# ideafisher/ssUnet-GAN

Hardware: AMD Instinct MI355X
Metric: train images/sec (512^2 tiles) (higher is better)
Workload: dtype f32; 1 GPU; UNet_R_SS_v2 generator + SRGAN-style discriminator, one G+D step (train_seg_gan.py:182-233), 16 x 3x512x512 tiles per GPU, fp32, Adam lr 2e-5; global_batch=16, tile=512, parallelism=dp1, dead_d_param_grads_of_g_step=computed

## Files before the change

ssunet-gan_amd/csrc/bn.hip:

```cpp
#include "common.h"

namespace {

constexpr int RED_BLOCK = 256;
constexpr int MAX_PARTS = 1024;

struct RedGeom { int TQ, PR, groups, parts; long long rows_per_part; };

__host__ RedGeom red_geom(long long P, int C, int Q = 1) {
  RedGeom g;
  const int CQ = (C + 4 * Q - 1) / (4 * Q);
  g.TQ = CQ >= 64 ? 64 : 1;
  if (CQ < 64) { while (g.TQ < CQ) g.TQ <<= 1; }
  g.PR = RED_BLOCK / g.TQ;
  g.groups = (CQ + g.TQ - 1) / g.TQ;
  long long parts = (P + (long long)g.PR * 8 - 1) / ((long long)g.PR * 8);
  if (parts > MAX_PARTS) parts = MAX_PARTS;
  if (parts < 1) parts = 1;
  g.rows_per_part = (P + parts - 1) / parts;
  g.parts = (int)((P + g.rows_per_part - 1) / g.rows_per_part);
  return g;
}

template <int MODE, typename T, bool BITS = false>
// ... 115 lines not shown
    double* dst = part + (size_t)blockIdx.x * 2 * Cpad;
#pragma unroll
    for (int e = 0; e < V; ++e) { dst[V * cg + e] = a1[e]; dst[Cpad + V * cg + e] = a2[e]; }
  }
}

__global__ __launch_bounds__(RED_BLOCK) void modulate_bwd_sums_kernel(
    const float* __restrict__ x, int ldx, const float* __restrict__ gb, int ldgb, const float* __restrict__ dy, int lddy,
    long long P, int C, float* __restrict__ dx, int lddx, float* __restrict__ dgb, int lddgb,
    int TQ, int PR, long long rows_per_part, double* __restrict__ part ) {
  __shared__ double red[2][RED_BLOCK][4];
  const int tid = threadIdx.x;
  const int tq = tid % TQ, pr = tid / TQ;
  const int cq = blockIdx.y * TQ + tq;
  const int CQ = C / 4;
  const bool cok = cq < CQ;
  const long long p0 = (long long)blockIdx.x * rows_per_part;
  long long p1 = p0 + rows_per_part; if (p1 > P) p1 = P;
  double s1[4] = {0, 0, 0, 0}, s2[4] = {0, 0, 0, 0};
  if (cok) {
    for (long long p = p0 + pr; p < p1; p += PR) {
      const f32x4 xv = *(const f32x4*)(x + p * ldx + 4 * cq);
      const f32x4 g = *(const f32x4*)(gb + p * ldgb + 4 * cq);
      const f32x4 d = *(const f32x4*)(dy + p * lddy + 4 * cq);
      const f32x4 dg = d * xv;
      st4(dx + p * lddx + 4 * cq, d * (1.f + g));
      st4(dgb + p * lddgb + 4 * cq, dg);
      st4(dgb + p * lddgb + C + 4 * cq, d);
#pragma unroll
      for (int e = 0; e < 4; ++e) { s1[e] += (double)dg[e]; s2[e] += (double)d[e]; }
    }
  }
#pragma unroll
  for (int e = 0; e < 4; ++e) { red[0][tid][e] = s1[e]; red[1][tid][e] = s2[e]; }
  __syncthreads();
  if (pr == 0 && cok) {
    double a1[4] = {0, 0, 0, 0}, a2[4] = {0, 0, 0, 0};
    for (int r = 0; r < PR; ++r)
#pragma unroll
      for (int e = 0; e < 4; ++e) { a1[e] += red[0][r * TQ + tq][e]; a2[e] += red[1][r * TQ + tq][e]; }
    double* dst = part + (size_t)blockIdx.x * 2 * C;
#pragma unroll
    for (int e = 0; e < 4; ++e) { dst[4 * cq + e] = a1[e]; dst[C + 4 * cq + e] = a2[e]; }
  }
}

__global__ __launch_bounds__(RED_BLOCK) void modulate_dgamma_sums_kernel(
    const float* __restrict__ x, int ldx, const float* __restrict__ dy, int lddy, long long P, int C,
    float* __restrict__ dg_out, int lddg, int TQ, int PR, long long rows_per_part, double* __restrict__ part ) {
  __shared__ double red[2][RED_BLOCK][4];
  const int tid = threadIdx.x;
  const int tq = tid % TQ, pr = tid / TQ;
  const int cq = blockIdx.y * TQ + tq;
  const int CQ = C / 4;
  const bool cok = cq < CQ;
  const long long p0 = (long long)blockIdx.x * rows_per_part;
  long long p1 = p0 + rows_per_part; if (p1 > P) p1 = P;
  double s1[4] = {0, 0, 0, 0}, s2[4] = {0, 0, 0, 0};
  if (cok) {
    for (long long p = p0 + pr; p < p1; p += PR) {
      const f32x4 xv = *(const f32x4*)(x + p * ldx + 4 * cq);
      const f32x4 d = *(const f32x4*)(dy + p * lddy + 4 * cq);
      const f32x4 dg = d * xv;
      st4(dg_out + p * lddg + 4 * cq, dg);
#pragma unroll
      for (int e = 0; e < 4; ++e) { s1[e] += (double)dg[e]; s2[e] += (double)d[e]; }
    }
  }
#pragma unroll
  for (int e = 0; e < 4; ++e) { red[0][tid][e] = s1[e]; red[1][tid][e] = s2[e]; }
  __syncthreads();
  if (pr == 0 && cok) {
    double a1[4] = {0, 0, 0, 0}, a2[4] = {0, 0, 0, 0};
    for (int r = 0; r < PR; ++r)
#pragma unroll
      for (int e = 0; e < 4; ++e) { a1[e] += red[0][r * TQ + tq][e]; a2[e] += red[1][r * TQ + tq][e]; }
    double* dst = part + (size_t)blockIdx.x * 2 * C;
#pragma unroll
    for (int e = 0; e < 4; ++e) { dst[4 * cq + e] = a1[e]; dst[C + 4 * cq + e] = a2[e]; }
  }
}

constexpr int FIN_LANES = 32;

struct BnFin {
  const float* weight; const float* bias; float eps, momentum; int var_mode;
  float* running_mean; float* running_var; float* mean; float* invstd; float* scale; float* shift;
};

__device__ __forceinline__ void bn_finalize_channel(int c, double s1, double s2, double count, const BnFin& f) {
  const double m = s1 / count;
  double var = fma(-m, m, s2 / count);
  if (var < 0) var = 0;
  double is;
  if (f.var_mode == 0) is = 1.0 / sqrt(var + (double)f.eps);
  else is = 1.0 / sqrt(var < (double)f.eps ? (double)f.eps : var);
  const float mf = (float)m, isf = (float)is;
  f.mean[c] = mf; f.invstd[c] = isf;
  const float w = f.weight ? f.weight[c] : 1.f, b = f.bias ? f.bias[c] : 0.f;
  const float sc = w * isf;
  f.scale[c] = sc; f.shift[c] = fmaf(-mf, sc, b);
  if (f.running_mean) f.running_mean[c] = fmaf(f.momentum, mf, (1.f - f.momentum) * f.running_mean[c]);
  if (f.running_var) {
    const double unb = count > 1 ? var * count / (count - 1) : var;
    f.running_var[c] = fmaf(f.momentum, (float)unb, (1.f - f.momentum) * f.running_var[c]);
  }
}

__global__ __launch_bounds__(32 * FIN_LANES) void col_reduce_final_kernel(const double* __restrict__ part, int parts, int C, int C4,
                                                                          double* __restrict__ sums, float* __restrict__ fsum,
                                                                          double count_out, BnFin fin, double fin_count) {
  __shared__ double red[2][FIN_LANES][32];
  const int cl = threadIdx.x & 31, lane = threadIdx.x >> 5;
  const int c = blockIdx.x * 32 + cl;
  double a1 = 0, a2 = 0;
  if (c < C) {
#pragma unroll 4
    for (int b = lane; b < parts; b += FIN_LANES) { a1 += part[(size_t)b * 2 * C4 + c]; a2 += part[(size_t)b * 2 * C4 + C4 + c]; }
  }
  red[0][lane][cl] = a1; red[1][lane][cl] = a2;
  __syncthreads();
  if (lane == 0 && c < C) {
    double t1 = 0, t2 = 0;
#pragma unroll
    for (int k = 0; k < FIN_LANES; ++k) { t1 += red[0][k][cl]; t2 += red[1][k][cl]; }
    if (sums) { sums[c] = t1; sums[C + c] = t2; }
    if (fsum) fsum[c] = (float)t1;
    if (fin.mean) bn_finalize_channel(c, t1, t2, fin_count, fin);
  }
  if (sums && count_out > 0 && blockIdx.x == 0 && threadIdx.x == 0) sums[2 * C] = count_out;
}

__global__ void bn_finalize_kernel(const double* __restrict__ sums, double count_arg, int C, BnFin fin) {
  const int c = blockIdx.x * blockDim.x + threadIdx.x;
  if (c >= C) return;
  const double count = count_arg > 0 ? count_arg : sums[2 * C];
  bn_finalize_channel(c, sums[c], sums[C + c], count, fin);
}

template <typename T>
__global__ __launch_bounds__(256) void bn_apply_kernel(const T* __restrict__ x, long long P, int C, int ld,
                                                       const float* __restrict__ scale, const float* __restrict__ shift,
                                                       const T* __restrict__ res, int ldr, int act, float slope,
                                                       T* __restrict__ y, int ldy) {
  constexpr int Q = SsgQ<T>::value;
  const int CG = C / (4 * Q);
  const long long total = P * CG;
  SSG_CHUNK_LOOP(i, total) {
    const long long p = i / CG; const int c0 = 4 * Q * (int)(i - p * CG);
    f32x4 xv[Q], rv[Q], o[Q];
    ldq(x + p * ld + c0, xv);
    if (res) ldq(res + p * ldr + c0, rv);
#pragma unroll
    for (int q = 0; q < Q; ++q) {
      const f32x4 sc = *(const f32x4*)(scale + c0 + 4 * q), sh = *(const f32x4*)(shift + c0 + 4 * q);
      f32x4 v = xv[q] * sc + sh;
      if (res) v += rv[q];
#pragma unroll
      for (int e = 0; e < 4; ++e) v[e] = ssg_act(v[e], act, slope);
      o[q] = v;
    }
    stq(y + p * ldy + c0, o);
  }
}

__global__ __launch_bounds__(256) void bn_apply_mask_kernel(const float* __restrict__ x, long long P, int C, int ld,
                                                            const float* __restrict__ scale, const float* __restrict__ shift,
                                                            const float* __restrict__ res, int ldr, int act, float slope,
                                                            float* __restrict__ y, int ldy, uint8_t* __restrict__ mask, int ldm) {
  const int CG = C / 4;
  const long long total = P * CG;
  SSG_CHUNK_LOOP(i, total) {
    const long long p = i / CG; const int cq = (int)(i - p * CG); const int c0 = 4 * cq;
    const f32x4 xv = *(const f32x4*)(x + p * ld + c0);
    f32x4 rv = f32x4{0.f, 0.f, 0.f, 0.f};
    if (res) rv = *(const f32x4*)(res + p * ldr + c0);
    const f32x4 sc = *(const f32x4*)(scale + c0), sh = *(const f32x4*)(shift + c0);
    f32x4 v = xv * sc + sh;
    if (res) v += rv;
    unsigned nib = 0;
#pragma unroll
    for (int e = 0; e < 4; ++e) {
      v[e] = ssg_act(v[e], act, slope);
      nib |= (v[e] > 0.f ? 1u : 0u) << e;
    }
    st4(y + p * ldy + c0, v);
    const unsigned other = (unsigned)__builtin_amdgcn_mov_dpp((int)nib, 0xB1, 0xf, 0xf, false);
    if (!(cq & 1)) mask[p * ldm + (cq >> 1)] = (uint8_t)(nib | (other << 4));
  }
}

__device__ __forceinline__ float bn_dx_elem(float g, float xv, double k_mean, double k_is, double k_ws, double k_m1, double k_m2) {
  const double xh = ((double)xv - k_mean) * k_is;
  return (float)(k_ws * fma(-xh, k_m2, (double)g - k_m1));
}
__device__ __forceinline__ float bn_dx_elem(float g, float xv, float k_mean, float k_is, float k_ws, float k_m1, float k_m2) {
  const float xh = (xv - k_mean) * k_is;
  return k_ws * fmaf(-xh, k_m2, g - k_m1);
}

template <typename T, bool BITS = false>
// ... 572 lines not shown
```

ssunet-gan_amd/csrc/conv_wgrad.hip:

```cpp
#include "common.h"
#include "conv_thin.h"
#include "conv_wgrad_args.h"

namespace {

constexpr int BKP = 16;

template <int BM, int BN, int WAVES_M, int WAVES_N>
__global__ __launch_bounds__(256) void wgrad_kernel(const WgArgs a) {
  constexpr int WTM = BM / WAVES_M, WTN = BN / WAVES_N;
  constexpr int MI = WTM / 32, NI = WTN / 32;
  constexpr int LDA = BM + 4, LDB = BN + 4;
  constexpr int AQ = BM / 4, BQ = BN / 4;
  constexpr int A_LD = BKP * AQ / 256, B_LD = (BKP * BQ + 255) / 256;
  constexpr int A_PSTEP = 256 / AQ, B_PSTEP = 256 / BQ;
  static_assert(A_LD >= 1, "tile");

  __shared__ __attribute__((aligned(16))) float lds[2 * BKP * (LDA + LDB)];
  float* As = lds;
  float* Bs = lds + 2 * BKP * LDA;

  const int tid = threadIdx.x, lane = tid & 63, wave = tid >> 6;
  const int wm = wave / WAVES_N, wn = wave % WAVES_N;
  const int half = lane >> 5, l31 = lane & 31;
// ... 53 lines not shown
  };

  f32x16 acc[MI][NI];
#pragma unroll
  for (int i = 0; i < MI; ++i)
#pragma unroll
    for (int j = 0; j < NI; ++j)
#pragma unroll
      for (int r = 0; r < 16; ++r) acc[i][j][r] = 0.f;

  if (nsteps > 0) {
    load_step(0);
    store_step(0);
  }
  __syncthreads();
  for (int s = 0; s < nsteps; ++s) {
    const int buf = s & 1;
    const bool more = (s + 1) < nsteps;
    if (more) load_step(s + 1);
    const float* Ab = As + buf * BKP * LDA + half * LDA + wm * WTM + l31;
    const float* Bb = Bs + buf * BKP * LDB + half * LDB + wn * WTN + l31;
#pragma unroll
    for (int kk = 0; kk < BKP / 2; ++kk) {
      float fa[MI], fb[NI];
#pragma unroll
      for (int i = 0; i < MI; ++i) fa[i] = Ab[2 * kk * LDA + i * 32];
#pragma unroll
      for (int j = 0; j < NI; ++j) fb[j] = Bb[2 * kk * LDB + j * 32];
#pragma unroll
      for (int i = 0; i < MI; ++i)
#pragma unroll
        for (int j = 0; j < NI; ++j)
          acc[i][j] = __builtin_amdgcn_mfma_f32_32x32x2f32(fa[i], fb[j], acc[i][j], 0, 0, 0);
    }
    if (more) store_step(buf ^ 1);
    __syncthreads();
  }

  float* slab = a.ws + (size_t)blockIdx.z * a.M * a.Cout;
#pragma unroll
  for (int i = 0; i < MI; ++i)
#pragma unroll
    for (int j = 0; j < NI; ++j) {
      const int co = n0 + wn * WTN + j * 32 + l31;
#pragma unroll
      for (int r = 0; r < 16; ++r) {
        const int row = m0 + wm * WTM + i * 32 + (r & 3) + 8 * (r >> 2) + 4 * half;
        if (row < a.M && co < a.Cout) slab[(size_t)row * a.Cout + co] = acc[i][j][r];
      }
    }
}

struct RedArgs {
  const float* ws; float* dw; int splits, M, Cout, Cin, Cin_real, KH, KW, ntaps;
  int ky[SSG_MAX_TAPS], kx[SSG_MAX_TAPS];
};

template <int ZL>
__global__ __launch_bounds__(32 * ZL) void wgrad_reduce_kernel(const RedArgs a) {
  __shared__ float red[ZL][32];
  const int el = threadIdx.x & 31, zl = threadIdx.x >> 5;
  const long long idx = (long long)blockIdx.x * 32 + el;
  const long long tot = (long long)a.M * a.Cout;
  float s = 0.f;
  if (idx < tot) {
    int z = zl;
    for (; z + 3 * ZL < a.splits; z += 4 * ZL) {
      const float v0 = a.ws[(size_t)z * tot + idx], v1 = a.ws[(size_t)(z + ZL) * tot + idx];
      const float v2 = a.ws[(size_t)(z + 2 * ZL) * tot + idx], v3 = a.ws[(size_t)(z + 3 * ZL) * tot + idx];
      s += v0; s += v1; s += v2; s += v3;
    }
    for (; z < a.splits; z += ZL) s += a.ws[(size_t)z * tot + idx];
  }
  red[zl][el] = s;
  __syncthreads();
  if (zl != 0 || idx >= tot) return;
  float v = 0.f;
#pragma unroll
  for (int k = 0; k < ZL; ++k) v += red[k][el];
  const int row = (int)(idx / a.Cout), co = (int)(idx - (long long)row * a.Cout);
  const int t = row / a.Cin, c = row - t * a.Cin;
  if (c >= a.Cin_real) return;
  a.dw[(((size_t)co * a.Cin_real + c) * a.KH + a.ky[t]) * a.KW + a.kx[t]] = v;
}

enum { WG_MFMA, WG_HALO, WG_K32, WG_4 };
struct Plan { int variant, mt, nt, splits, steps_per_split, kind; };

bool wgrad_uses_dma(int variant) { return variant <= 1; }

bool wgrad_uses_halo(const ssg_wgrad_desc* d, int variant) { return wgrad_uses_dma(variant) && ssg_wgrad_halo_ok(d, variant); }

Plan make_plan(const ssg_wgrad_desc* d) {
  Plan p;
  p.kind = WG_MFMA;
  if (const int w4 = ssg_wgrad4_kind(d)) {
    p.kind = WG_4; p.variant = w4;
    p.mt = p.nt = p.steps_per_split = 0;
    p.splits = ssg_wgrad4_slices(d, w4, nullptr, nullptr, nullptr);
    return p;
  }
  const int Cin = d->C1 + d->C2;
  const int M = d->ntaps * Cin;
  int bn;
  if (d->Cout > 64) { p.variant = 0; bn = 128; }
  else if (d->Cout > 32) { p.variant = 1; bn = 64; }
  else { p.variant = 2; bn = 32; }
  p.mt = (M + 127) / 128;
  p.nt = (d->Cout + bn - 1) / bn;
  long long steps = ((long long)d->N * d->GH * d->GW + BKP - 1) / BKP;
  if (wgrad_uses_halo(d, p.variant)) {
    p.kind = WG_HALO;
    p.mt = Cin / ssg_wgrad_halo_cb(p.variant);
    steps = (long long)d->N * d->GH * ((d->GW + BKP - 1) / BKP);
  }
  if ((d->flags & 1) && ssg_wgrad_k32_ok(d)) {
    p.kind = WG_K32;
    p.mt = Cin / 64; p.nt = d->Cout / 64;
    steps = ssg_wgrad_k32_steps(d);
    const long long tiles = (long long)p.mt * p.nt;
    long long max_rows = 128;
    {
      const long long steps16 = (long long)d->N * d->GH * ((d->GW + BKP - 1) / BKP);
      const long long mtf = Cin / ssg_wgrad_halo_cb(p.variant), ntf = (d->Cout + (p.variant == 0 ? 127 : 63)) / (p.variant == 0 ? 128 : 64);
      long long wantf = 1024 / (mtf * ntf > 0 ? mtf * ntf : 1);
      if (wantf < 1) wantf = 1;
      if (wantf > steps16 / 16) wantf = steps16 / 16 > 0 ? steps16 / 16 : 1;
      if (wantf > 512) wantf = 512;
      const long long chain_px = (steps16 + wantf - 1) / wantf * BKP;
      if (chain_px / 32 < max_rows) max_rows = chain_px / 32;
      if (max_rows < 8) max_rows = 8;
    }
    const WgSlabs s = ssg_wgrad_slabs(steps, tiles, 8, max_rows);
    p.steps_per_split = s.steps_per_split; p.splits = s.splits;
    return p;
  }
  long long want = 1024 / ((long long)p.mt * p.nt);
  if (want < 1) want = 1;
  long long maxs = steps / 16;
  if (maxs < 1) maxs = 1;
  if (want > maxs) want = maxs;
  if (want > 512) want = 512;
  p.steps_per_split = (int)((steps + want - 1) / want);
  p.splits = (int)((steps + p.steps_per_split - 1) / p.steps_per_split);
  return p;
}

int validate(const ssg_wgrad_desc* d) {
  SSG_REQUIRE(d && d->in1 && d->dout && d->dw_oihw, SSG_EINVAL, "wgrad: null pointer");
  SSG_REQUIRE(d->C1 > 0 && d->C1 % 4 == 0 && d->C2 >= 0 && d->C2 % 4 == 0, SSG_EINVAL, "wgrad: channels must be multiples of 4");
  SSG_REQUIRE(d->C2 == 0 || d->in2, SSG_EINVAL, "wgrad: C2 > 0 needs in2");
  SSG_REQUIRE(d->ld1 % 4 == 0 && d->ld1 >= d->C1 && d->ldd % 4 == 0 && d->ldd >= d->Cout, SSG_EALIGN, "wgrad: strides");
  SSG_REQUIRE(d->C2 == 0 || (d->ld2 % 4 == 0 && d->ld2 >= d->C2), SSG_EALIGN, "wgrad: ld2");
  SSG_REQUIRE(ssg_aligned16(d->in1) && ssg_aligned16(d->in2) && ssg_aligned16(d->dout) && ssg_aligned16(d->ws), SSG_EALIGN, "wgrad: alignment");
  SSG_REQUIRE(d->ntaps >= 1 && d->ntaps <= SSG_MAX_TAPS, SSG_EINVAL, "wgrad: ntaps");
  SSG_REQUIRE(d->Cin_real > 0 && d->Cin_real <= d->C1 + d->C2, SSG_EINVAL, "wgrad: Cin_real");
  for (int t = 0; t < d->ntaps; ++t) {
    SSG_REQUIRE(d->dy[t] >= -2 && d->dy[t] <= 5 && d->dx[t] >= -2 && d->dx[t] <= 5, SSG_EINVAL, "wgrad: tap offset");
    SSG_REQUIRE(d->ky[t] >= 0 && d->ky[t] < d->KH && d->kx[t] >= 0 && d->kx[t] < d->KW, SSG_EINVAL, "wgrad: kernel position");
  }
  return SSG_OK;
}

int64_t workspace_bytes(const ssg_wgrad_desc* d, const Plan& p) {
  return (int64_t)p.splits * d->ntaps * (d->C1 + d->C2) * d->Cout * (int64_t)sizeof(float);
}
// ... 15 lines not shown
    const int span = ntaps * 16;
    const int chunk = k / span, rem = k - chunk * span;
    t = rem >> 4; c = chunk * 16 + (rem & 15);
  } else {
    t = k / Cred_pad; c = k - t * Cred_pad;
  }
  const int Cred = transpose ? O : I;
  float v = 0.f;
  if (t < ntaps && c < Cred) {
    const int kb = (int)((kpos_bits >> (6 * t)) & 63ull);
    const int ky = kb & 7, kx = kb >> 3;
    const int o = transpose ? c : r, i = transpose ? r : c;
    v = w[(((size_t)o * I + i) * KH + ky) * KW + kx];
    if (sigma) v *= 1.f / *sigma;
  }
  out[idx] = v;
}

}

WgArgs ssg_wgrad_args(const ssg_wgrad_desc* d, int steps_per_split) {
  WgArgs a;
  a.in1 = d->in1; a.in2 = d->C2 ? d->in2 : d->in1; a.dout = d->dout; a.ws = d->ws;
  a.C1 = d->C1; a.C2 = d->C2; a.ld1 = d->ld1; a.ld2 = d->C2 ? d->ld2 : d->ld1;
  a.N = d->N; a.H = d->H; a.W = d->W; a.Cout = d->Cout; a.ldd = d->ldd; a.GH = d->GH; a.GW = d->GW;
  a.in_sy = d->in_sy; a.in_sx = d->in_sx; a.ntaps = d->ntaps;
  a.tap_bits = ssg_pack_taps(d->dy, d->dx, d->ntaps);
  a.in_scale = d->in_scale; a.in_shift = d->in_shift; a.in_act = d->in_act; a.in_slope = d->in_slope;
  a.M = d->ntaps * (d->C1 + d->C2);
  a.Ptot = (long long)d->N * d->GH * d->GW;
  a.steps_per_split = steps_per_split;
  a.xcd_swizzle = 0;
  return a;
}

extern "C" int64_t ssg_conv2d_wgrad_workspace_bytes(const ssg_wgrad_desc* d) {
  return d ? workspace_bytes(d, make_plan(d)) : 0;
}

extern "C" int ssg_conv2d_wgrad_in_affine_ok(const ssg_wgrad_desc* d) {
  if (!d || !d->in1 || !d->dout) return 0;
  return in_affine_ok(d, make_plan(d)) ? 1 : 0;
}

extern "C" int ssg_conv2d_wgrad_f32(const ssg_wgrad_desc* d, void* stream) {
  int rc = validate(d);
  if (rc != SSG_OK) return rc;
  const Plan p = make_plan(d);
  SSG_REQUIRE(d->ws_bytes >= workspace_bytes(d, p), SSG_EINVAL, "wgrad: workspace too small");
  SSG_REQUIRE(!d->in_scale || (d->in_shift && in_affine_ok(d, p)), SSG_EINVAL,
              "wgrad: in_scale on a descriptor whose kernel has no fused input transform (ssg_conv2d_wgrad_in_affine_ok == 0)");
  hipStream_t st = (hipStream_t)stream;
  WgArgs a = ssg_wgrad_args(d, p.steps_per_split);
  if (p.kind == WG_4) {
    rc = ssg_wgrad4_launch(d, p.variant, st);
    if (rc != SSG_OK) return rc;
  } else {
    dim3 grid((unsigned)p.mt, (unsigned)p.nt, (unsigned)p.splits);
    if (p.kind == WG_K32) {
      rc = ssg_wgrad_k32_launch(a, grid, st);
      if (rc != SSG_OK) return rc;
    } else if (p.kind == WG_HALO) {
      rc = ssg_wgrad_halo_launch(a, p.variant, grid, st, (d->flags & 1) != 0);
      if (rc != SSG_OK) return rc;
    } else if (wgrad_uses_dma(p.variant)) {
      rc = ssg_wgrad_dma_launch(a, p.variant, grid, st, (d->flags & 1) != 0);
      if (rc != SSG_OK) return rc;
    } else {
      hipLaunchKernelGGL((wgrad_kernel<128, 32, 4, 1>), grid, dim3(256), 0, st, a);
    }
    SSG_LAUNCH_CHECK();
  }
  return ssg_wgrad_reduce_launch(d, p.splits, st);
}

int ssg_wgrad_reduce_launch(const ssg_wgrad_desc* d, int splits, hipStream_t st) {
  RedArgs r;
  r.ws = d->ws; r.dw = d->dw_oihw; r.splits = splits; r.M = d->ntaps * (d->C1 + d->C2); r.Cout = d->Cout; r.Cin = d->C1 + d->C2;
  r.Cin_real = d->Cin_real; r.KH = d->KH; r.KW = d->KW; r.ntaps = d->ntaps;
  for (int t = 0; t < SSG_MAX_TAPS; ++t) { r.ky[t] = t < d->ntaps ? d->ky[t] : 0; r.kx[t] = t < d->ntaps ? d->kx[t] : 0; }
  const long long tot = (long long)r.M * d->Cout;
  if (splits >= 256 && tot <= 32 * 1024)
    hipLaunchKernelGGL(wgrad_reduce_kernel<32>, dim3((unsigned)ssg_cdiv(tot, 32)), dim3(1024), 0, st, r);
  else
    hipLaunchKernelGGL(wgrad_reduce_kernel<8>, dim3((unsigned)ssg_cdiv(tot, 32)), dim3(256), 0, st, r);
  SSG_LAUNCH_CHECK();
  return SSG_OK;
}

extern "C" int ssg_pack_weights_scaled_f32(const float* w_oihw, int O, int I, int KH, int KW, int transpose, int ntaps,
                                           const int* ky, const int* kx, int kmode, int Cred_pad, int Kp, const float* sigma, float* out,
                                           void* stream);
extern "C" int ssg_pack_weights_f32(const float* w_oihw, int O, int I, int KH, int KW, int transpose, int ntaps,
                                    const int* ky, const int* kx, int kmode, int Cred_pad, int Kp, float* out,
                                    void* stream) {
  return ssg_pack_weights_scaled_f32(w_oihw, O, I, KH, KW, transpose, ntaps, ky, kx, kmode, Cred_pad, Kp, nullptr, out, stream);
}
extern "C" int ssg_pack_weights_scaled_f32(const float* w_oihw, int O, int I, int KH, int KW, int transpose, int ntaps,
                                           const int* ky, const int* kx, int kmode, int Cred_pad, int Kp, const float* sigma, float* out,
                                           void* stream) {
  SSG_REQUIRE(w_oihw && out && ky && kx, SSG_EINVAL, "pack: null pointer");
  SSG_REQUIRE(ntaps >= 1 && ntaps <= SSG_MAX_TAPS && KH <= 8 && KW <= 8, SSG_EINVAL, "pack: taps");
  SSG_REQUIRE(Kp % 16 == 0 && Cred_pad % 4 == 0, SSG_EINVAL, "pack: Kp/Cred_pad");
  const int Cred = transpose ? O : I;
  SSG_REQUIRE(Cred_pad >= Cred, SSG_EINVAL, "pack: Cred_pad < reduced channels");
  if (kmode == 0) SSG_REQUIRE(Cred_pad % 16 == 0 && Kp == ntaps * Cred_pad, SSG_EINVAL, "pack: kmode 0 shape");
  else SSG_REQUIRE(Kp >= ntaps * Cred_pad, SSG_EINVAL, "pack: kmode 1 Kp");
  unsigned long long bits = 0;
  for (int t = 0; t < ntaps; ++t) {
    SSG_REQUIRE(ky[t] >= 0 && ky[t] < KH && kx[t] >= 0 && kx[t] < KW, SSG_EINVAL, "pack: kernel position");
    bits |= (unsigned long long)(ky[t] | (kx[t] << 3)) << (6 * t);
  }
  const int R = transpose ? I : O;
  const long long tot = (long long)R * Kp;
  hipLaunchKernelGGL(pack_weights_kernel, dim3((unsigned)ssg_cdiv(tot, 256)), dim3(256), 0, (hipStream_t)stream,
                     w_oihw, O, I, KH, KW, transpose, ntaps, bits, kmode, Cred_pad, Kp, R, out, sigma);
  SSG_LAUNCH_CHECK();
  return SSG_OK;
}

extern "C" int ssg_conv2d_wgrad_kernel_id(const ssg_wgrad_desc* d) {
  if (!d) return SSG_EINVAL;
  const Plan p = make_plan(d);
  if (p.kind == WG_4) return 10 + p.variant;
  if (p.kind == WG_K32) return 60;
  if (p.kind == WG_HALO) return ((d->flags & 1) ? 40 : 30) + p.variant;
  return p.variant + (wgrad_uses_dma(p.variant) ? ((d->flags & 1) ? 50 : 20) : 0);
}

extern "C" int ssg_wgrad_dma_body(const ssg_wgrad_desc* d) {
  if (!d || validate(d) != SSG_OK) return 0;
  const Plan p = make_plan(d);
  if (p.kind != WG_MFMA || !wgrad_uses_dma(p.variant) || !(d->flags & 1)) return 0;
  return ssg_wgrad_dma_split_body(ssg_wgrad_args(d, p.steps_per_split), p.variant, (long long)p.mt * p.nt * p.splits);
}
```

ssunet-gan_amd/csrc/spatial.hip:

```cpp
#include "common.h"

namespace {

int elem_grid(long long total) { return ssg_elem_grid(total, 2); }

#define GRID_STRIDE(i, total) SSG_CHUNK_LOOP(i, total)

__global__ __launch_bounds__(256) void maxpool_fwd_kernel(const float* __restrict__ x, int N, int H, int W, int C, int ldx,
                                                          float* __restrict__ y, int ldy, uint8_t* __restrict__ idx) {
  const int OH = H / 2, OW = W / 2, CQ = C / 4;
  const long long total = (long long)N * OH * OW * CQ;
  GRID_STRIDE(i, total) {
    const int cq = (int)(i % CQ); long long r = i / CQ;
    const int ox = (int)(r % OW); r /= OW;
    const int oy = (int)(r % OH); const int n = (int)(r / OH);
    const float* b = x + ((size_t)(n * H + 2 * oy) * W + 2 * ox) * ldx + 4 * cq;
    f32x4 best = *(const f32x4*)b;
    int bi[4] = {0, 0, 0, 0};
#pragma unroll
    for (int k = 1; k < 4; ++k) {
      const f32x4 v = *(const f32x4*)(b + ((size_t)(k >> 1) * W + (k & 1)) * ldx);
#pragma unroll
      for (int e = 0; e < 4; ++e)
        if (v[e] > best[e] || v[e] != v[e]) { best[e] = v[e]; bi[e] = k; }
// ... 185 lines not shown
  int xlo, xhi;
  cand_range(ix, sx, OW, xlo, xhi);
  int oxf = -1, cnt = 0; float wx[5] = {0.f, 0.f, 0.f, 0.f, 0.f};
  for (int ox = xlo; ox <= xhi; ++ox) {
    int x0, x1; float lx0, lx1;
    lerp_coord(ox, sx, W, x0, x1, lx0, lx1);
    if (x0 != ix && x1 != ix) continue;
    if (oxf < 0) oxf = ox;
    const float wgt = (x0 == ix ? lx0 : 0.f) + (x1 == ix ? lx1 : 0.f);
    const int k = ox - oxf;
    if (k < 5) cnt = k + 1;
#pragma unroll
    for (int q = 0; q < 5; ++q) if (q == k) wx[q] = wgt;
  }
  const int b0 = band * BIL_BWD_BAND, b1 = min(b0 + BIL_BWD_BAND, H);
  int oylo, oyhi, t;
  cand_range(b0, sy, OH, oylo, t);
  cand_range(b1 - 1, sy, OH, t, oyhi);
  const float* src = dy + ((size_t)n * OH * OW + (oxf < 0 ? 0 : oxf)) * lddy + c4;
  float* dst = dx + ((size_t)n * H * W + ix) * lddx + c4;
  auto flush = [&](int r, const f32x4& v) { if (r >= b0 && r < b1) *(f32x4*)(dst + (size_t)r * W * lddx) = v; };
  int y0, y1; float ly0, ly1;
  lerp_coord(oylo, sy, H, y0, y1, ly0, ly1);
  int cur = y0;
  f32x4 acc0 = {0, 0, 0, 0}, acc1 = {0, 0, 0, 0};
  for (int oy = oylo; oy <= oyhi; ++oy) {
    lerp_coord(oy, sy, H, y0, y1, ly0, ly1);
    const float* row = src + (size_t)oy * OW * lddy;
    f32x4 h = {0, 0, 0, 0};
#pragma unroll
    for (int q = 0; q < 5; ++q)
      if (q < cnt) h += wx[q] * *(const f32x4*)(row + (size_t)q * lddy);
    if (y0 > cur) { flush(cur, acc0); acc0 = acc1; acc1 = f32x4{0, 0, 0, 0}; cur = y0; }
    acc0 += ly0 * h;
    if (y1 != y0) acc1 += ly1 * h; else acc0 += ly1 * h;
  }
  flush(cur, acc0);
  flush(cur + 1, acc1);
}

__global__ __launch_bounds__(256) void nearest_fwd_kernel(const float* __restrict__ x, int N, int H, int W, int C, int ldx,
                                                          float* __restrict__ y, int ldy) {
  const int OH = 2 * H, OW = 2 * W, CQ = C / 4;
  const long long total = (long long)N * OH * OW * CQ;
  GRID_STRIDE(i, total) {
    const int cq = (int)(i % CQ); long long r = i / CQ;
    const int ox = (int)(r % OW); r /= OW;
    const int oy = (int)(r % OH); const int n = (int)(r / OH);
    *(f32x4*)(y + ((size_t)(n * OH + oy) * OW + ox) * ldy + 4 * cq) =
        *(const f32x4*)(x + ((size_t)(n * H + (oy >> 1)) * W + (ox >> 1)) * ldx + 4 * cq);
  }
}
__global__ __launch_bounds__(256) void nearest_bwd_kernel(const float* __restrict__ dy, int lddy, int N, int H, int W, int C,
                                                          float* __restrict__ dx, int lddx) {
  const int OW = 2 * W, CQ = C / 4;
  const long long total = (long long)N * H * W * CQ;
  GRID_STRIDE(i, total) {
    const int cq = (int)(i % CQ); long long r = i / CQ;
    const int ix = (int)(r % W); r /= W;
    const int iy = (int)(r % H); const int n = (int)(r / H);
    const float* b = dy + ((size_t)(n * 2 * H + 2 * iy) * OW + 2 * ix) * lddy + 4 * cq;
    const f32x4 s = (*(const f32x4*)b + *(const f32x4*)(b + lddy)) + (*(const f32x4*)(b + (size_t)OW * lddy) + *(const f32x4*)(b + (size_t)(OW + 1) * lddy));
    *(f32x4*)(dx + ((size_t)(n * H + iy) * W + ix) * lddx + 4 * cq) = s;
  }
}

__device__ __forceinline__ int bin_lo(int o, int in, int out) { return (o * in) / out; }
__device__ __forceinline__ int bin_hi(int o, int in, int out) { return ((o + 1) * in + out - 1) / out; }

__global__ __launch_bounds__(256) void avgpool_flat_fwd_kernel(const float* __restrict__ x, int N, int H, int W, int C, int ldx,
                                                               int O, float* __restrict__ y) {
  const long long total = (long long)N * O * O * C;
  GRID_STRIDE(i, total) {
    const int c = (int)(i % C); long long r = i / C;
    const int ox = (int)(r % O); r /= O;
    const int oy = (int)(r % O); const int n = (int)(r / O);
    const int y0 = bin_lo(oy, H, O), y1 = bin_hi(oy, H, O), x0 = bin_lo(ox, W, O), x1 = bin_hi(ox, W, O);
    float s = 0.f;
    for (int yy = y0; yy < y1; ++yy)
      for (int xx = x0; xx < x1; ++xx) s += x[((size_t)(n * H + yy) * W + xx) * ldx + c];
    y[(size_t)n * C * O * O + (size_t)c * O * O + oy * O + ox] = s / (float)((y1 - y0) * (x1 - x0));
  }
}
__global__ __launch_bounds__(256) void avgpool_flat_bwd_kernel(const float* __restrict__ dy, int N, int H, int W, int C, int O,
                                                               float* __restrict__ dx, int lddx) {
  const long long total = (long long)N * H * W * C;
  GRID_STRIDE(i, total) {
    const int c = (int)(i % C); long long r = i / C;
    const int xx = (int)(r % W); r /= W;
    const int yy = (int)(r % H); const int n = (int)(r / H);
    float s = 0.f;
    for (int oy = 0; oy < O; ++oy) {
      const int y0 = bin_lo(oy, H, O), y1 = bin_hi(oy, H, O);
      if (yy < y0 || yy >= y1) continue;
      for (int ox = 0; ox < O; ++ox) {
        const int x0 = bin_lo(ox, W, O), x1 = bin_hi(ox, W, O);
        if (xx < x0 || xx >= x1) continue;
        s += dy[(size_t)n * C * O * O + (size_t)c * O * O + oy * O + ox] / (float)((y1 - y0) * (x1 - x0));
      }
    }
    dx[((size_t)(n * H + yy) * W + xx) * lddx + c] = s;
  }
}

__global__ __launch_bounds__(256) void nchw_to_nhwc_kernel(const float* __restrict__ src, int C, long long S, float* __restrict__ dst, int ld) {
  const long long p = (long long)blockIdx.x * 64 + (threadIdx.x & 63);
  const int n = blockIdx.y;
  if (p >= S) return;
  for (int c = threadIdx.x >> 6; c < ld; c += 4) {
    const float v = c < C ? src[((size_t)n * C + c) * S + p] : 0.f;
    dst[((size_t)n * S + p) * ld + c] = v;
  }
}
__global__ __launch_bounds__(256) void nhwc_to_nchw_kernel(const float* __restrict__ src, int ld, int C, long long S, float* __restrict__ dst) {
  const long long p = (long long)blockIdx.x * 64 + (threadIdx.x & 63);
  const int n = blockIdx.y;
  if (p >= S) return;
  for (int c = threadIdx.x >> 6; c < C; c += 4) dst[((size_t)n * C + c) * S + p] = src[((size_t)n * S + p) * ld + c];
}

static bool bilinear_stream_ok(int N, int H, int W, int C) {
  return C % 16 == 0 && H >= 3 && W >= 3 && (long long)N * (2 * H / BIL_FWD_BAND + 1) * (2 * W / 16 + 1) * (C / 16) < (1ll << 31);
}
#define REQ_Q(C, ...) SSG_REQUIRE((C) > 0 && (C) % 4 == 0, SSG_EINVAL, __VA_ARGS__)

}

extern "C" int ssg_maxpool2x2_fwd_f32(const float* x, int N, int H, int W, int C, int ldx, float* y, int ldy, uint8_t* idx, void* stream) {
  SSG_REQUIRE(x && y && idx && N > 0 && H >= 2 && W >= 2, SSG_EINVAL, "maxpool: bad args");
  REQ_Q(C, "maxpool: C %% 4");
  SSG_REQUIRE(ldx % 4 == 0 && ldy % 4 == 0, SSG_EALIGN, "maxpool: strides");
  const long long total = (long long)N * (H / 2) * (W / 2) * (C / 4);
  hipLaunchKernelGGL(maxpool_fwd_kernel, dim3(elem_grid(total)), dim3(256), 0, (hipStream_t)stream, x, N, H, W, C, ldx, y, ldy, idx);
  SSG_LAUNCH_CHECK();
  return SSG_OK;
}
extern "C" int ssg_maxpool2x2_bwd_f32(const float* dy, int lddy, const uint8_t* idx, int N, int H, int W, int C, float* dx, int lddx, void* stream) {
  SSG_REQUIRE(dy && dx && idx && N > 0 && H % 2 == 0 && W % 2 == 0, SSG_EINVAL, "maxpool_bwd: needs even H, W");
  REQ_Q(C, "maxpool_bwd: C %% 4");
  const long long total = (long long)N * (H / 2) * (W / 2) * (C / 4);
  hipLaunchKernelGGL(scatter2x2_kernel, dim3(elem_grid(total)), dim3(256), 0, (hipStream_t)stream, dy, lddy, idx, N, H / 2, W / 2, C, dx, lddx, (const float*)nullptr, 0);
  SSG_LAUNCH_CHECK();
  return SSG_OK;
}
extern "C" int ssg_maxpool2x2_bwd_add_f32(const float* dy, int lddy, const uint8_t* idx, const float* res, int ldr, int N, int H, int W, int C,
                                         float* dx, int lddx, void* stream) {
  SSG_REQUIRE(dy && dx && idx && res && N > 0 && H % 2 == 0 && W % 2 == 0 && ldr % 4 == 0, SSG_EINVAL, "maxpool_bwd_add: bad args");
  REQ_Q(C, "maxpool_bwd_add: C %% 4");
  const long long total = (long long)N * (H / 2) * (W / 2) * (C / 4);
  hipLaunchKernelGGL(scatter2x2_kernel, dim3(elem_grid(total)), dim3(256), 0, (hipStream_t)stream, dy, lddy, idx, N, H / 2, W / 2, C, dx, lddx, res, ldr);
  SSG_LAUNCH_CHECK();
  return SSG_OK;
}
extern "C" int ssg_maxunpool2x2_fwd_f32(const float* x, int ldx, const uint8_t* idx, int N, int OH, int OW, int C, float* y, int ldy, void* stream) {
  SSG_REQUIRE(x && y && idx && N > 0 && OH % 2 == 0 && OW % 2 == 0, SSG_EINVAL, "maxunpool: bad args");
  REQ_Q(C, "maxunpool: C %% 4");
  const long long total = (long long)N * (OH / 2) * (OW / 2) * (C / 4);
  hipLaunchKernelGGL(scatter2x2_kernel, dim3(elem_grid(total)), dim3(256), 0, (hipStream_t)stream, x, ldx, idx, N, OH / 2, OW / 2, C, y, ldy, (const float*)nullptr, 0);
  SSG_LAUNCH_CHECK();
  return SSG_OK;
}
extern "C" int ssg_maxunpool2x2_bwd_f32(const float* dy, int lddy, const uint8_t* idx, int N, int OH, int OW, int C, float* dx, int lddx, void* stream) {
  SSG_REQUIRE(dy && dx && idx && N > 0 && OH % 2 == 0 && OW % 2 == 0, SSG_EINVAL, "maxunpool_bwd: bad args");
  REQ_Q(C, "maxunpool_bwd: C %% 4");
  const long long total = (long long)N * (OH / 2) * (OW / 2) * (C / 4);
  hipLaunchKernelGGL(gather2x2_kernel, dim3(elem_grid(total)), dim3(256), 0, (hipStream_t)stream, dy, lddy, idx, N, OH / 2, OW / 2, C, dx, lddx);
  SSG_LAUNCH_CHECK();
  return SSG_OK;
}
extern "C" int ssg_upsample2x_bilinear_fwd_f32(const float* x, int N, int H, int W, int C, int ldx, float* y, int ldy, void* stream) {
  SSG_REQUIRE(x && y && N > 0 && H > 0 && W > 0, SSG_EINVAL, "bilinear: bad args");
  REQ_Q(C, "bilinear: C %% 4");
  const float sy = (2 * H > 1) ? (float)(H - 1) / (float)(2 * H - 1) : 0.f, sx = (2 * W > 1) ? (float)(W - 1) / (float)(2 * W - 1) : 0.f;
  SSG_REQUIRE((long long)N * 2 * H < (1ll << 31) && (long long)2 * W * (C / 4) < (1ll << 31), SSG_EINVAL, "bilinear: too large");
  if (bilinear_stream_ok(N, H, W, C)) {
    const int cqt = C % 64 == 0 ? 16 : C % 32 == 0 ? 8 : 4;
    const int nct = C / (4 * cqt), ncb = (2 * W + 256 / cqt - 1) / (256 / cqt), nb = (2 * H + BIL_FWD_BAND - 1) / BIL_FWD_BAND;
    const dim3 grid((unsigned)((long long)N * nb * ncb * nct));
    if (cqt == 16) hipLaunchKernelGGL(bilinear_fwd_stream_kernel<16>, grid, dim3(256), 0, (hipStream_t)stream, x, N, H, W, C, ldx, y, ldy, sy, sx, nct, ncb, nb);
    else if (cqt == 8) hipLaunchKernelGGL(bilinear_fwd_stream_kernel<8>, grid, dim3(256), 0, (hipStream_t)stream, x, N, H, W, C, ldx, y, ldy, sy, sx, nct, ncb, nb);
    else hipLaunchKernelGGL(bilinear_fwd_stream_kernel<4>, grid, dim3(256), 0, (hipStream_t)stream, x, N, H, W, C, ldx, y, ldy, sy, sx, nct, ncb, nb);
    SSG_LAUNCH_CHECK();
    return SSG_OK;
  }
  const unsigned cols = (unsigned)(2 * W) * (unsigned)(C / 4);
  const unsigned gy = cols / 1024 ? (cols / 1024 > 64 ? 64 : cols / 1024) : 1;
  SSG_REQUIRE((long long)N * 2 * H * gy < (1ll << 31), SSG_EINVAL, "bilinear: too large");
  hipLaunchKernelGGL(bilinear_fwd_kernel, dim3((unsigned)(N * 2 * H) * gy), dim3(256), 0, (hipStream_t)stream, x, N, H, W, C, ldx, y, ldy, sy, sx, gy);
  SSG_LAUNCH_CHECK();
  return SSG_OK;
}
extern "C" int ssg_upsample2x_bilinear_bwd_f32(const float* dy, int lddy, int N, int H, int W, int C, float* dx, int lddx, void* stream) {
  SSG_REQUIRE(dy && dx && N > 0 && H > 0 && W > 0, SSG_EINVAL, "bilinear_bwd: bad args");
  REQ_Q(C, "bilinear_bwd: C %% 4");
  const float sy = (2 * H > 1) ? (float)(H - 1) / (float)(2 * H - 1) : 0.f, sx = (2 * W > 1) ? (float)(W - 1) / (float)(2 * W - 1) : 0.f;
  SSG_REQUIRE((long long)N * H < (1ll << 31) && (long long)W * (C / 4) < (1ll << 31), SSG_EINVAL, "bilinear_bwd: too large");
  if (bilinear_stream_ok(N, H, W, C)) {
    const int cqt = C % 64 == 0 ? 16 : C % 32 == 0 ? 8 : 4;
    const int nct = C / (4 * cqt), ncb = (W + 256 / cqt - 1) / (256 / cqt), nb = (H + BIL_BWD_BAND - 1) / BIL_BWD_BAND;
    const dim3 grid((unsigned)((long long)N * nb * ncb * nct));
    if (cqt == 16) hipLaunchKernelGGL(bilinear_bwd_stream_kernel<16>, grid, dim3(256), 0, (hipStream_t)stream, dy, lddy, N, H, W, C, dx, lddx, sy, sx, nct, ncb, nb);
    else if (cqt == 8) hipLaunchKernelGGL(bilinear_bwd_stream_kernel<8>, grid, dim3(256), 0, (hipStream_t)stream, dy, lddy, N, H, W, C, dx, lddx, sy, sx, nct, ncb, nb);
    else hipLaunchKernelGGL(bilinear_bwd_stream_kernel<4>, grid, dim3(256), 0, (hipStream_t)stream, dy, lddy, N, H, W, C, dx, lddx, sy, sx, nct, ncb, nb);
    SSG_LAUNCH_CHECK();
    return SSG_OK;
  }
  const unsigned cols = (unsigned)W * (unsigned)(C / 4);
  const unsigned gy = (cols + 255) / 256 > 64 ? 64 : (cols + 255) / 256;
  SSG_REQUIRE((long long)N * H * gy < (1ll << 31), SSG_EINVAL, "bilinear_bwd: too large");
  hipLaunchKernelGGL(bilinear_bwd_kernel, dim3((unsigned)(N * H) * gy), dim3(256), 0, (hipStream_t)stream, dy, lddy, N, H, W, C, dx, lddx, sy, sx, gy);
  SSG_LAUNCH_CHECK();
  return SSG_OK;
}
extern "C" int ssg_upsample2x_nearest_fwd_f32(const float* x, int N, int H, int W, int C, int ldx, float* y, int ldy, void* stream) {
  SSG_REQUIRE(x && y && N > 0 && H > 0 && W > 0, SSG_EINVAL, "nearest: bad args");
  REQ_Q(C, "nearest: C %% 4");
  const long long total = (long long)N * 4 * H * W * (C / 4);
  hipLaunchKernelGGL(nearest_fwd_kernel, dim3(elem_grid(total)), dim3(256), 0, (hipStream_t)stream, x, N, H, W, C, ldx, y, ldy);
  SSG_LAUNCH_CHECK();
  return SSG_OK;
}
extern "C" int ssg_upsample2x_nearest_bwd_f32(const float* dy, int lddy, int N, int H, int W, int C, float* dx, int lddx, void* stream) {
  SSG_REQUIRE(dy && dx && N > 0 && H > 0 && W > 0, SSG_EINVAL, "nearest_bwd: bad args");
  REQ_Q(C, "nearest_bwd: C %% 4");
  const long long total = (long long)N * H * W * (C / 4);
  hipLaunchKernelGGL(nearest_bwd_kernel, dim3(elem_grid(total)), dim3(256), 0, (hipStream_t)stream, dy, lddy, N, H, W, C, dx, lddx);
  SSG_LAUNCH_CHECK();
  return SSG_OK;
}
extern "C" int ssg_adaptive_avgpool_flat_fwd_f32(const float* x, int N, int H, int W, int C, int ldx, int OHW, float* y, void* stream) {
  SSG_REQUIRE(x && y && N > 0 && H > 0 && W > 0 && C > 0 && OHW > 0, SSG_EINVAL, "avgpool: bad args");
  const long long total = (long long)N * OHW * OHW * C;
  hipLaunchKernelGGL(avgpool_flat_fwd_kernel, dim3(elem_grid(total)), dim3(256), 0, (hipStream_t)stream, x, N, H, W, C, ldx, OHW, y);
  SSG_LAUNCH_CHECK();
  return SSG_OK;
}
extern "C" int ssg_adaptive_avgpool_flat_bwd_f32(const float* dy, int N, int H, int W, int C, int OHW, float* dx, int lddx, void* stream) {
  SSG_REQUIRE(dy && dx && N > 0 && H > 0 && W > 0 && C > 0 && OHW > 0, SSG_EINVAL, "avgpool_bwd: bad args");
  const long long total = (long long)N * H * W * C;
  hipLaunchKernelGGL(avgpool_flat_bwd_kernel, dim3(elem_grid(total)), dim3(256), 0, (hipStream_t)stream, dy, N, H, W, C, OHW, dx, lddx);
  SSG_LAUNCH_CHECK();
  return SSG_OK;
}
extern "C" int ssg_nchw_to_nhwc_f32(const float* src, int N, int C, int H, int W, float* dst, int ld, void* stream) {
  SSG_REQUIRE(src && dst && N > 0 && C > 0 && ld >= C, SSG_EINVAL, "nchw_to_nhwc: bad args");
  const long long S = (long long)H * W;
  hipLaunchKernelGGL(nchw_to_nhwc_kernel, dim3((unsigned)ssg_cdiv(S, 64), (unsigned)N), dim3(256), 0, (hipStream_t)stream, src, C, S, dst, ld);
  SSG_LAUNCH_CHECK();
  return SSG_OK;
}
extern "C" int ssg_nhwc_to_nchw_f32(const float* src, int ld, int N, int C, int H, int W, float* dst, void* stream) {
  SSG_REQUIRE(src && dst && N > 0 && C > 0 && ld >= C, SSG_EINVAL, "nhwc_to_nchw: bad args");
  const long long S = (long long)H * W;
  hipLaunchKernelGGL(nhwc_to_nchw_kernel, dim3((unsigned)ssg_cdiv(S, 64), (unsigned)N), dim3(256), 0, (hipStream_t)stream, src, ld, C, S, dst);
  SSG_LAUNCH_CHECK();
  return SSG_OK;
}
```

Before: 90.46 images/sec.

## Speed up BN final reduce, few-split wgrad reduce, and avgpool backward

Three independent kernel changes. The BN column-reduce final kernel batches eight partial loads per lane before accumulating, so more memory requests are in flight. A new vectorized wgrad split-reduce kernel handles the few-split, large-tensor case with float4 loads and a compile-time unrolled split count. Adaptive avgpool backward now computes only the overlapping output bins, vectorizes over channels, and adds an LDS-staged variant for small pooled sizes. The cost is more code paths and more template instantiations.

```diff
diff --git a/ssunet-gan_amd/csrc/bn.hip b/ssunet-gan_amd/csrc/bn.hip
--- a/ssunet-gan_amd/csrc/bn.hip
+++ b/ssunet-gan_amd/csrc/bn.hip
@@ -221,6 +221,7 @@
 }
 
 constexpr int FIN_LANES = 32;
+constexpr int FIN_U = 8;
 
 struct BnFin {
   const float* weight; const float* bias; float eps, momentum; int var_mode;
@@ -254,8 +255,17 @@
   const int c = blockIdx.x * 32 + cl;
   double a1 = 0, a2 = 0;
   if (c < C) {
-#pragma unroll 4
-    for (int b = lane; b < parts; b += FIN_LANES) { a1 += part[(size_t)b * 2 * C4 + c]; a2 += part[(size_t)b * 2 * C4 + C4 + c]; }
+    for (int b = lane; b < parts; b += FIN_LANES * FIN_U) {
+      double v1[FIN_U], v2[FIN_U];
+#pragma unroll
+      for (int u = 0; u < FIN_U; ++u) {
+        const int bb = b + FIN_LANES * u;
+        if (bb < parts) { v1[u] = part[(size_t)bb * 2 * C4 + c]; v2[u] = part[(size_t)bb * 2 * C4 + C4 + c]; }
+      }
+#pragma unroll
+      for (int u = 0; u < FIN_U; ++u)
+        if (b + FIN_LANES * u < parts) { a1 += v1[u]; a2 += v2[u]; }
+    }
   }
   red[0][lane][cl] = a1; red[1][lane][cl] = a2;
   __syncthreads();
diff --git a/ssunet-gan_amd/csrc/conv_wgrad.hip b/ssunet-gan_amd/csrc/conv_wgrad.hip
--- a/ssunet-gan_amd/csrc/conv_wgrad.hip
+++ b/ssunet-gan_amd/csrc/conv_wgrad.hip
@@ -159,6 +159,43 @@
   const int t = row / a.Cin, c = row - t * a.Cin;
   if (c >= a.Cin_real) return;
   a.dw[(((size_t)co * a.Cin_real + c) * a.KH + a.ky[t]) * a.KW + a.kx[t]] = v;
+}
+
+constexpr int RED_FEW = 48;
+constexpr long long RED_FEW_MIN = 576 * 1024, RED_FEW_MAX = 4096 * 1024;
+template <int NB>
+__global__ __launch_bounds__(256) void wgrad_reduce_few_kernel(const RedArgs a) {
+  constexpr int ZL = 8;
+  const long long idx = ((long long)blockIdx.x * 256 + threadIdx.x) * 4;
+  const long long tot = (long long)a.M * a.Cout;
+  if (idx >= tot) return;
+  const float* p = a.ws + idx;
+  const int zr = (a.splits - 1) % ZL;
+  f32x4 v = {0.f, 0.f, 0.f, 0.f};
+#pragma unroll
+  for (int z = 0; z < ZL; ++z) {
+    const bool whole = z <= zr;
+    f32x4 q[NB];
+#pragma unroll
+    for (int u = 0; u < NB - 1; ++u) q[u] = *(const f32x4*)(p + (size_t)(z + u * ZL) * tot);
+    if (whole) q[NB - 1] = *(const f32x4*)(p + (size_t)(z + (NB - 1) * ZL) * tot);
+    f32x4 s = {0.f, 0.f, 0.f, 0.f};
+#pragma unroll
+    for (int u = 0; u < NB - 1; ++u) s += q[u];
+    if (whole) s += q[NB - 1];
+    v += s;
+  }
+  const int row = (int)(idx / a.Cout), co = (int)(idx - (long long)row * a.Cout);
+  const int t = row / a.Cin, c = row - t * a.Cin;
+  if (c >= a.Cin_real) return;
+  const size_t ostride = (size_t)a.Cin_real * a.KH * a.KW;
+  float* o = a.dw + (((size_t)co * a.Cin_real + c) * a.KH + a.ky[t]) * a.KW + a.kx[t];
+#pragma unroll
+  for (int e = 0; e < 4; ++e) o[e * ostride] = v[e];
+}
+template <int NB>
+void reduce_few_launch(const RedArgs& r, long long tot, hipStream_t st) {
+  hipLaunchKernelGGL(wgrad_reduce_few_kernel<NB>, dim3((unsigned)ssg_cdiv(tot, 1024)), dim3(256), 0, st, r);
 }
 
 enum { WG_MFMA, WG_HALO, WG_K32, WG_4 };
@@ -340,10 +377,29 @@
   const long long tot = (long long)r.M * d->Cout;
   if (splits >= 256 && tot <= 32 * 1024)
     hipLaunchKernelGGL(wgrad_reduce_kernel<32>, dim3((unsigned)ssg_cdiv(tot, 32)), dim3(1024), 0, st, r);
-  else
+  else if (splits <= RED_FEW && tot >= RED_FEW_MIN && tot <= RED_FEW_MAX && d->Cout % 4 == 0 && ssg_aligned16(d->ws)) {
+    switch ((splits + 7) / 8) {
+      case 1: reduce_few_launch<1>(r, tot, st); break;
+      case 2: reduce_few_launch<2>(r, tot, st); break;
+      case 3: reduce_few_launch<3>(r, tot, st); break;
+      case 4: reduce_few_launch<4>(r, tot, st); break;
+      case 5: reduce_few_launch<5>(r, tot, st); break;
+      case 6: reduce_few_launch<6>(r, tot, st); break;
+      case 7: reduce_few_launch<7>(r, tot, st); break;
+      default: reduce_few_launch<8>(r, tot, st); break;
+    }
+  } else
     hipLaunchKernelGGL(wgrad_reduce_kernel<8>, dim3((unsigned)ssg_cdiv(tot, 32)), dim3(256), 0, st, r);
   SSG_LAUNCH_CHECK();
   return SSG_OK;
+}
+
+extern "C" int ssg_wgrad_reduce_only(const ssg_wgrad_desc* d, void* stream) {
+  const int rc = validate(d);
+  if (rc != SSG_OK) return rc;
+  const Plan p = make_plan(d);
+  SSG_REQUIRE(d->ws_bytes >= workspace_bytes(d, p), SSG_EINVAL, "wgrad: workspace too small");
+  return ssg_wgrad_reduce_launch(d, p.splits, (hipStream_t)stream);
 }
 
 extern "C" int ssg_pack_weights_scaled_f32(const float* w_oihw, int O, int I, int KH, int KW, int transpose, int ntaps,
diff --git a/ssunet-gan_amd/csrc/spatial.hip b/ssunet-gan_amd/csrc/spatial.hip
--- a/ssunet-gan_amd/csrc/spatial.hip
+++ b/ssunet-gan_amd/csrc/spatial.hip
@@ -291,24 +291,59 @@
     y[(size_t)n * C * O * O + (size_t)c * O * O + oy * O + ox] = s / (float)((y1 - y0) * (x1 - x0));
   }
 }
+template <int V>
 __global__ __launch_bounds__(256) void avgpool_flat_bwd_kernel(const float* __restrict__ dy, int N, int H, int W, int C, int O,
                                                                float* __restrict__ dx, int lddx) {
-  const long long total = (long long)N * H * W * C;
-  GRID_STRIDE(i, total) {
-    const int c = (int)(i % C); long long r = i / C;
+  const int CG = C / V, OO = O * O;
+  const long long total = (long long)N * H * W * CG;
+  GRID_STRIDE(i, total) {
+    const int c = V * (int)(i % CG); long long r = i / CG;
     const int xx = (int)(r % W); r /= W;
     const int yy = (int)(r % H); const int n = (int)(r / H);
-    float s = 0.f;
-    for (int oy = 0; oy < O; ++oy) {
+    const int oy0 = (yy * O) / H, oy1 = ((yy + 1) * O - 1) / H, ox0 = (xx * O) / W, ox1 = ((xx + 1) * O - 1) / W;
+    const float* b = dy + ((size_t)n * C + c) * OO;
+    float s[V];
+#pragma unroll
+    for (int e = 0; e < V; ++e) s[e] = 0.f;
+    for (int oy = oy0; oy <= oy1; ++oy) {
       const int y0 = bin_lo(oy, H, O), y1 = bin_hi(oy, H, O);
-      if (yy < y0 || yy >= y1) continue;
-      for (int ox = 0; ox < O; ++ox) {
+      for (int ox = ox0; ox <= ox1; ++ox) {
         const int x0 = bin_lo(ox, W, O), x1 = bin_hi(ox, W, O);
-        if (xx < x0 || xx >= x1) continue;
-        s += dy[(size_t)n * C * O * O + (size_t)c * O * O + oy * O + ox] / (float)((y1 - y0) * (x1 - x0));
+        const float area = (float)((y1 - y0) * (x1 - x0));
+#pragma unroll
+        for (int e = 0; e < V; ++e) s[e] += b[e * OO + oy * O + ox] / area;
       }
     }
-    dx[((size_t)(n * H + yy) * W + xx) * lddx + c] = s;
+    float* o = dx + ((size_t)(n * H + yy) * W + xx) * lddx + c;
+    if constexpr (V == 4) st4(o, f32x4{s[0], s[1], s[2], s[3]});
+    else o[0] = s[0];
+  }
+}
+constexpr int POOL_CG = 64, POOL_PX = 256;
+__global__ __launch_bounds__(256) void avgpool_flat_bwd_staged_kernel(const float* __restrict__ dy, int H, int W, int C, int O,
+                                                                      float* __restrict__ dx, int lddx) {
+  __shared__ __attribute__((aligned(16))) float sd[64][POOL_CG + 4];
+  const int n = blockIdx.z, c0 = blockIdx.y * POOL_CG, OO = O * O, HW = H * W;
+  const float* src = dy + ((size_t)n * C + c0) * OO;
+  for (int j = threadIdx.x; j < POOL_CG * OO; j += 256) sd[j % OO][j / OO] = src[j];
+  __syncthreads();
+  const int cq = threadIdx.x & 15;
+  int p1 = (blockIdx.x + 1) * POOL_PX; if (p1 > HW) p1 = HW;
+  for (int px = blockIdx.x * POOL_PX + (threadIdx.x >> 4); px < p1; px += 16) {
+    const int yy = px / W, xx = px - yy * W;
+    const int oy0 = (yy * O) / H, oy1 = ((yy + 1) * O - 1) / H, ox0 = (xx * O) / W, ox1 = ((xx + 1) * O - 1) / W;
+    float s[4] = {0.f, 0.f, 0.f, 0.f};
+    for (int oy = oy0; oy <= oy1; ++oy) {
+      const int y0 = bin_lo(oy, H, O), y1 = bin_hi(oy, H, O);
+      for (int ox = ox0; ox <= ox1; ++ox) {
+        const int x0 = bin_lo(ox, W, O), x1 = bin_hi(ox, W, O);
+        const float area = (float)((y1 - y0) * (x1 - x0));
+        const f32x4 g = *(const f32x4*)&sd[oy * O + ox][4 * cq];
+#pragma unroll
+        for (int e = 0; e < 4; ++e) s[e] += g[e] / area;
+      }
+    }
+    st4(dx + ((size_t)n * HW + px) * lddx + c0 + 4 * cq, f32x4{s[0], s[1], s[2], s[3]});
   }
 }
 
@@ -446,8 +481,14 @@
 }
 extern "C" int ssg_adaptive_avgpool_flat_bwd_f32(const float* dy, int N, int H, int W, int C, int OHW, float* dx, int lddx, void* stream) {
   SSG_REQUIRE(dy && dx && N > 0 && H > 0 && W > 0 && C > 0 && OHW > 0, SSG_EINVAL, "avgpool_bwd: bad args");
-  const long long total = (long long)N * H * W * C;
-  hipLaunchKernelGGL(avgpool_flat_bwd_kernel, dim3(elem_grid(total)), dim3(256), 0, (hipStream_t)stream, dy, N, H, W, C, OHW, dx, lddx);
+  const bool quads = C % 4 == 0 && lddx % 4 == 0 && ssg_aligned16(dx);
+  if (quads && C % POOL_CG == 0 && OHW <= 8 && N <= 65535 && (long long)H * W < (1ll << 30))
+    hipLaunchKernelGGL(avgpool_flat_bwd_staged_kernel, dim3((unsigned)ssg_cdiv((long long)H * W, POOL_PX), (unsigned)(C / POOL_CG), (unsigned)N),
+                       dim3(256), 0, (hipStream_t)stream, dy, H, W, C, OHW, dx, lddx);
+  else if (quads)
+    hipLaunchKernelGGL(avgpool_flat_bwd_kernel<4>, dim3(elem_grid((long long)N * H * W * (C / 4))), dim3(256), 0, (hipStream_t)stream, dy, N, H, W, C, OHW, dx, lddx);
+  else
+    hipLaunchKernelGGL(avgpool_flat_bwd_kernel<1>, dim3(elem_grid((long long)N * H * W * C)), dim3(256), 0, (hipStream_t)stream, dy, N, H, W, C, OHW, dx, lddx);
   SSG_LAUNCH_CHECK();
   return SSG_OK;
 }
```

New measurement: 90.61 images/sec, median of 3. About the same (+0.2%).
